# PathologyFoundation/plip

Hardware: NVIDIA H100
Metric: image-text pairs/sec (224x224, 77-tok) (higher is better)
Workload: dtype bf16

## Files before the change

include/plip_b200.h:

```cpp
#ifndef PLIP_B200_H_
#define PLIP_B200_H_

#include <stdint.h>

#ifdef __cplusplus
extern "C" {
#endif

#define PLIP_API __attribute__((visibility("default")))

#define PLIP_B200_ABI_VERSION 5

#define PLIP_IMAGE_SIZE 224
#define PLIP_EMBED_DIM 512
#define PLIP_TEXT_SEQ 77
#define PLIP_VOCAB 49408

typedef struct plip_engine plip_engine_t;

enum plip_pixel_format {
  PLIP_PIX_F32_NCHW = 0,
  PLIP_PIX_BF16_NCHW = 1,
  PLIP_PIX_U8_NHWC = 2
};
// ... 130 lines not shown

typedef struct plip_densenet plip_densenet_t;
PLIP_API int plip_densenet_num_tensors(void);
PLIP_API int plip_densenet_tensor_info(int index, plip_tensor_info_t* info);
PLIP_API uint64_t plip_densenet_blob_bytes(void);
PLIP_API uint64_t plip_densenet_workspace_bytes(int max_micro_batch);
PLIP_API int plip_densenet_create(const void* host_blob, uint64_t blob_bytes, int device, int max_micro_batch,
                                  plip_densenet_t** out);
PLIP_API int plip_densenet_destroy(plip_densenet_t* e);
PLIP_API int plip_densenet_max_micro_batch(const plip_densenet_t* e);
PLIP_API int plip_densenet_encode(plip_densenet_t* e, const void* tiles_dev, int64_t n, float* out_dev, void* stream);

PLIP_API int plip_encode_images_host(plip_engine_t* e, const void* pixels_host, int pixel_format, int64_t n,
                                     float* out_host, int normalize);
PLIP_API int plip_encode_text_host(plip_engine_t* e, const void* ids_host, int ids_dtype,
                                   const void* attention_mask_host, int64_t n, int seq_len,
                                   float* out_host, int normalize);

typedef struct plip_kernel_time {
  char name[48];
  int32_t launches;
  float total_ms;
  double flops;
  double bytes;
} plip_kernel_time_t;
PLIP_API int plip_profile_enable(plip_engine_t* e, int on);
PLIP_API int plip_profile_read(plip_engine_t* e, plip_kernel_time_t* out, int cap, int* count);

PLIP_API int plip_dbg_set_operand_format(int operand_format);
PLIP_API int plip_dbg_gemm(const void* A_bf16, int lda, const void* W_bf16, int ldw, int M, int N, int K,
                           const float* bias, void* out, int ldo, const float* pos, int epilogue, int cluster_size,
                           int block_n, const float* colsum, const float* stats_in, int n_partials, void* xb_out,
                           float* stats_out, void* stream);
PLIP_API int plip_dbg_resize_filter(int in_size, int out_size, int xx, int32_t* k_host, int k_cap, int* xmin,
                                    int* count);
PLIP_API int plip_dbg_resize_filter_bilinear(int in_size, int out_size, int xx, int32_t* k_host, int k_cap, int* xmin,
                                             int* count);
PLIP_API int plip_dbg_text_bucket_plan(const int32_t* lens_host, int64_t n, int seq_len, int32_t* perm_host,
                                       int32_t* bucket_start_host, int32_t* bucket_prefix_host, int cap);
PLIP_API int plip_dbg_rowstats_cast(const float* x, int64_t rows, int dim, void* xb_bf16, float* stats, void* stream);
PLIP_API int plip_dbg_layernorm(const float* x, int64_t rows, int dim, int64_t in_row_stride,
                                const float* gamma, const float* beta, float* out_f32, void* out_bf16,
                                void* stream);
PLIP_API int plip_dbg_attention(const void* qkv_bf16, int64_t n_seq, int seq_len, int heads, int causal,
                                const int32_t* key_mask, void* out_bf16, void* stream);
PLIP_API int plip_dbg_attention_probs(const void* qkv_bf16, int64_t n_seq, int seq_len, int heads, int causal,
                                      const int32_t* key_mask, float* probs_dev, void* stream);
PLIP_API int plip_dbg_densenet_op(int op, const void* in_dev, int lda, int64_t n, int side, int c_in, const void* w_dev,
                                  const float* a_scale, const float* a_shift, const float* e_scale,
                                  const float* e_shift, void* out_dev, int ldo, void* stream);
PLIP_API int plip_dbg_im2col(const void* pixels, int pixel_format, int64_t n, void* out_bf16, void* stream);
PLIP_API int plip_dbg_pos_interp(const float* pos_dev, int grid_h, int grid_w, float* out_dev, void* stream);
PLIP_API int plip_dbg_hidden_states_hw(plip_engine_t* e, const void* pixels_dev, int pixel_format, int64_t n,
                                       int height, int width, int num_layers, float* hidden_dev, void* stream);
PLIP_API int plip_dbg_hidden_states(plip_engine_t* e, int tower, const void* input_dev, int input_format,
                                    const void* attention_mask_dev, int64_t n, int num_layers,
                                    float* hidden_dev, void* stream);

#ifdef __cplusplus
}
#endif
#endif
```

plip_b200/_lib.py:

```python
from __future__ import annotations

import ctypes as C
from pathlib import Path

_PKG = Path(__file__).resolve().parent
LIB_PATH = _PKG / "libplip_b200.so"

_vp = C.c_void_p
_i = C.c_int
_i64 = C.c_int64
_u64 = C.c_uint64
_f = C.c_float
_fp = C.c_void_p


class TensorInfo(C.Structure):

    _fields_ = [
        ("name", C.c_char * 96),
        ("offset", C.c_uint64),
        ("numel", C.c_uint64),
        ("dtype", C.c_int32),
        ("rows", C.c_int32),
        ("cols", C.c_int32),
# ... 62 lines not shown
    "plip_window_background_counts": (_i, [_vp, _i, _i, _i64, _vp, _i64, _i, _vp, _vp]),
    "plip_encode_text": (_i, [_vp, _vp, _i, _vp, _i64, _i, _fp, _i, _vp]),
    "plip_encode_text_prefix": (_i, [_vp, _vp, _i, _vp, _i64, _i, _i, _fp, _i, _vp]),
    "plip_vision_outputs": (_i, [_vp, _vp, _i, _i64, _i, _i, C.POINTER(TowerOutputs), _vp]),
    "plip_text_outputs": (_i, [_vp, _vp, _i, _vp, _i64, _i, C.POINTER(TowerOutputs), _vp]),
    "plip_similarity": (_i, [_fp, _i64, _fp, _i64, _f, _i, _i, _fp, _i64, _vp]),
    "plip_similarity_topk": (_i, [_fp, _i64, _fp, _i64, _f, _i, _i, _i, _vp, _fp, _vp]),
    "plip_l2_normalize": (_i, [_fp, _i64, _i, _vp]),
    "plip_window_mask_counts": (_i, [_vp, _i, _i, _i, _i64, _vp, _i64, _i, _vp, _vp]),
    "plip_resize_crop_u8": (_i, [_vp, _u64, _vp, _i64, _vp, _vp]),
    "plip_resize_crop_bilinear_u8": (_i, [_vp, _u64, _vp, _i64, _vp, _vp]),
    "plip_warp_tiles_u8": (_i, [_vp, _vp, _vp, _i64, _vp]),
    "plip_resize_region_workspace": (_i, [_i, _i, _i, _i, _i, _i, C.POINTER(_u64)]),
    "plip_resize_region_u8": (_i, [_vp, _i64, _i, _i, _i, _i, _vp, _i64, _i, _i, _i, _i, _vp, _u64, _vp]),
    "plip_resize_filter_bounds": (_i, [_i, _i, _vp]),
    "plip_sgd_shuffle_permutation": (_i, [_i64, C.c_uint32, _vp]),
    "plip_sgd_workspace_bytes": (_i, [_i64, _i, _i, C.POINTER(_u64)]),
    "plip_sgd_fit": (_i, [_fp, _i64, _i, _vp, _i, _vp, _i, _vp, _i, _i, C.c_double, _i, _fp, _vp, _vp, _vp, _vp, _u64,
                          _vp]),
    "plip_linear_decision": (_i, [_fp, _i64, _i, _fp, _vp, _i, _fp, _vp, _vp]),
    "plip_densenet_num_tensors": (_i, []),
    "plip_densenet_tensor_info": (_i, [_i, C.POINTER(TensorInfo)]),
    "plip_densenet_blob_bytes": (_u64, []),
    "plip_densenet_workspace_bytes": (_u64, [_i]),
    "plip_densenet_create": (_i, [_vp, _u64, _i, _i, C.POINTER(_vp)]),
    "plip_densenet_destroy": (_i, [_vp]),
    "plip_densenet_max_micro_batch": (_i, [_vp]),
    "plip_densenet_encode": (_i, [_vp, _vp, _i64, _fp, _vp]),
    "plip_encode_images_host": (_i, [_vp, _vp, _i, _i64, _fp, _i]),
    "plip_encode_text_host": (_i, [_vp, _vp, _i, _vp, _i64, _i, _fp, _i]),
    "plip_profile_enable": (_i, [_vp, _i]),
    "plip_profile_read": (_i, [_vp, C.POINTER(KernelTime), _i, C.POINTER(_i)]),
    "plip_dbg_gemm": (_i, [_vp, _i, _vp, _i, _i, _i, _i, _fp, _vp, _i, _fp, _i, _i, _i, _fp, _fp, _i, _vp, _fp, _vp]),
    "plip_dbg_resize_filter": (_i, [_i, _i, _i, _vp, _i, C.POINTER(_i), C.POINTER(_i)]),
    "plip_dbg_resize_filter_bilinear": (_i, [_i, _i, _i, _vp, _i, C.POINTER(_i), C.POINTER(_i)]),
    "plip_dbg_text_bucket_plan": (_i, [_vp, _i64, _i, _vp, _vp, _vp, _i]),
    "plip_dbg_rowstats_cast": (_i, [_fp, _i64, _i, _vp, _fp, _vp]),
    "plip_dbg_layernorm": (_i, [_fp, _i64, _i, _i64, _fp, _fp, _fp, _vp, _vp]),
    "plip_dbg_attention": (_i, [_vp, _i64, _i, _i, _i, _vp, _vp, _vp]),
    "plip_dbg_attention_probs": (_i, [_vp, _i64, _i, _i, _i, _vp, _fp, _vp]),
    "plip_dbg_densenet_op": (_i, [_i, _vp, _i, _i64, _i, _i, _vp, _fp, _fp, _fp, _fp, _vp, _i, _vp]),
    "plip_dbg_im2col": (_i, [_vp, _i, _i64, _vp, _vp]),
    "plip_dbg_hidden_states": (_i, [_vp, _i, _vp, _i, _vp, _i64, _i, _fp, _vp]),
    "plip_dbg_pos_interp": (_i, [_fp, _i, _i, _fp, _vp]),
    "plip_dbg_hidden_states_hw": (_i, [_vp, _vp, _i, _i64, _i, _i, _i, _fp, _vp]),
}

_LIB = None


def lib(strict: bool = True) -> C.CDLL:
    global _LIB
    if _LIB is not None:
        return _LIB
    if not LIB_PATH.exists():
        raise RuntimeError(
            f"{LIB_PATH} is missing: build it with `python -m plip_b200.build` "
            "(plip_b200 has no CPU fallback; the sm_90a CUDA library is the product)."
        )
    dll = C.CDLL(str(LIB_PATH))
    missing = []
    for name, (res, args) in SIGNATURES.items():
        try:
            fn = getattr(dll, name)
        except AttributeError:
            missing.append(name)
# ... 18 lines not shown
```

plip_b200/csrc/engine.cu:

```cuda
#include "kernels.cuh"

#include <stdlib.h>
#include <string.h>

#include <array>
#include <map>
#include <string>
#include <tuple>
#include <vector>

namespace plip {
const char* get_last_error();

namespace {

struct Spec {
  std::string name;
  int dtype;
  int rows, cols, fused;
  uint64_t offset, numel;
};

void add(std::vector<Spec>& v, const std::string& name, int dtype, int rows, int cols, int fused = 0) {
  Spec s;
// ... 1216 lines not shown
  }
  for (int k = 0; k < nb; ++k) {
    const int64_t r0 = start[k], cnt = start[k + 1] - start[k];
    if (cnt <= 0) continue;
    if (int rc = plip_encode_text_prefix(e, d_ids + (size_t)r0 * row_bytes, ids_dtype,
                                         d_mask ? d_mask + (size_t)r0 * row_bytes : nullptr, cnt, seq_len, prefix[k],
                                         e->d_out + r0 * kProj, normalize, e->s_compute)) return rc;
  }
  std::vector<float> tmp((size_t)n * kProj);
  PLIP_CUDA_CHECK(cudaMemcpyAsync(tmp.data(), e->d_out, (size_t)n * kProj * 4, cudaMemcpyDeviceToHost, e->s_compute));
  PLIP_CUDA_CHECK(cudaStreamSynchronize(e->s_compute));
  for (int64_t i = 0; i < n; ++i)
    memcpy(out_host + (size_t)perm[(size_t)i] * kProj, tmp.data() + (size_t)i * kProj, (size_t)kProj * 4);
  return 0;
}

PLIP_API int plip_dbg_text_bucket_plan(const int32_t* lens_host, int64_t n, int seq_len, int32_t* perm_host,
                                       int32_t* bucket_start_host, int32_t* bucket_prefix_host, int cap) {
  if (!lens_host || !bucket_start_host || !bucket_prefix_host || n <= 0 || seq_len < 1 || seq_len > kTxtSeq || cap < 1) {
    set_last_error("plip_dbg_text_bucket_plan: bad argument");
    return -2;
  }
  return plan_text_buckets(lens_host, n, seq_len, perm_host, bucket_start_host, bucket_prefix_host, cap);
}

static int g_dbg_f16 = 0;
PLIP_API int plip_dbg_set_operand_format(int operand_format) {
  PLIP_REQUIRE(operand_format == PLIP_OPERAND_BF16 || operand_format == PLIP_OPERAND_FP16,
               "plip_dbg_set_operand_format: unknown operand format %d", operand_format);
  g_dbg_f16 = operand_format == PLIP_OPERAND_FP16 ? 1 : 0;
  return 0;
}

PLIP_API int plip_dbg_gemm(const void* A_bf16, int lda, const void* W_bf16, int ldw, int M, int N, int K,
                           const float* bias, void* out, int ldo, const float* pos, int epilogue, int cluster_size,
                           int block_n, const float* colsum, const float* stats_in, int n_partials, void* xb_out,
                           float* stats_out, void* stream) {
  GemmArgs g;
  g.A = static_cast<const __nv_bfloat16*>(A_bf16); g.lda = lda;
  g.W = static_cast<const __nv_bfloat16*>(W_bf16); g.ldw = ldw;
  g.M = M; g.N = N; g.K = K;
  g.bias = bias; g.out = out; g.ldo = ldo; g.pos = pos; g.epi = epilogue;
  g.colsum = colsum; g.stats_in = reinterpret_cast<const float2*>(stats_in); g.n_partials = n_partials;
  g.xb_out = static_cast<__nv_bfloat16*>(xb_out); g.stats_out = reinterpret_cast<float2*>(stats_out);
  g.force_cg = cluster_size; g.force_bn = block_n;
  g.f16 = g_dbg_f16;
  return launch_gemm(g, static_cast<cudaStream_t>(stream));
}

PLIP_API int plip_dbg_rowstats_cast(const float* x, int64_t rows, int dim, void* xb_bf16, float* stats, void* stream) {
  return launch_rowstats_cast(x, rows, dim, static_cast<__nv_bfloat16*>(xb_bf16), reinterpret_cast<float2*>(stats),
                              g_dbg_f16, static_cast<cudaStream_t>(stream));
}

PLIP_API int plip_dbg_layernorm(const float* x, int64_t rows, int dim, int64_t in_row_stride, const float* gamma,
                                const float* beta, float* out_f32, void* out_bf16, void* stream) {
  return launch_layernorm(x, nullptr, in_row_stride, rows, dim, gamma, beta, out_f32,
                          static_cast<__nv_bfloat16*>(out_bf16), g_dbg_f16, static_cast<cudaStream_t>(stream));
}

PLIP_API int plip_dbg_attention(const void* qkv_bf16, int64_t n_seq, int seq_len, int heads, int causal,
                                const int32_t* key_mask, void* out_bf16, void* stream) {
  return launch_attention(static_cast<const __nv_bfloat16*>(qkv_bf16), n_seq, seq_len, heads, causal != 0, key_mask,
                          static_cast<__nv_bfloat16*>(out_bf16), g_dbg_f16, static_cast<cudaStream_t>(stream));
}

PLIP_API int plip_dbg_attention_probs(const void* qkv_bf16, int64_t n_seq, int seq_len, int heads, int causal,
                                      const int32_t* key_mask, float* probs_dev, void* stream) {
  return launch_attention_probs(static_cast<const __nv_bfloat16*>(qkv_bf16), n_seq, seq_len, heads, causal != 0,
                                key_mask, probs_dev, g_dbg_f16, static_cast<cudaStream_t>(stream));
}

PLIP_API int plip_dbg_im2col(const void* pixels, int pixel_format, int64_t n, void* out_bf16, void* stream) {
  return launch_im2col(pixels, pixel_format, n, kImage, kImage, static_cast<__nv_bfloat16*>(out_bf16), g_dbg_f16,
                       static_cast<cudaStream_t>(stream));
}

PLIP_API int plip_dbg_pos_interp(const float* pos_dev, int grid_h, int grid_w, float* out_dev, void* stream) {
  return launch_pos_interp(pos_dev, grid_h, grid_w, out_dev, static_cast<cudaStream_t>(stream));
}
// ... 16 lines not shown
```

plip_b200/csrc/gemm.cuh:

```cuda
#pragma once
#include "common.cuh"

namespace plip {

enum GemmEpilogue : int {
  EPI_BIAS_BF16 = 0,
  EPI_BIAS_GELU_BF16 = 1,
  EPI_BIAS_RESID_F32 = 2,
  EPI_PATCH_F32 = 3,
  EPI_F32 = 4,
  EPI_LN_BIAS_BF16 = 5,
  EPI_LN_BIAS_GELU_BF16 = 6,
  EPI_NULL = 7,
  EPI_SIM_F32 = 8,
  EPI_COUNT = 9
};

constexpr int kStatSlots = 8;

struct GemmArgs {
  const __nv_bfloat16* A = nullptr;
  int lda = 0;
  const __nv_bfloat16* W = nullptr;
  int ldw = 0;
  int M = 0, N = 0, K = 0;
  const float* bias = nullptr;
  const float* rowscale = nullptr;
  void* out = nullptr;
  int ldo = 0;
  const float* pos = nullptr;
  int patches = kPatches;
  int seq = kVisSeq;
  const float* colsum = nullptr;
  const float2* stats_in = nullptr;
  int n_partials = 0;
  __nv_bfloat16* xb_out = nullptr;
  float2* stats_out = nullptr;
  int* n_tiles_used = nullptr;
  int epi = EPI_F32;
  int f16 = 0;
  int force_cg = 0;
  int force_bn = 0;
};

int launch_gemm(const GemmArgs& g, cudaStream_t stream);

}
```

plip_b200/csrc/gemm_wgmma.cu:

```cuda
#include "gemm.cuh"
#include "wgmma.cuh"

#include <stdio.h>
#include <stdlib.h>

namespace plip {

namespace {

constexpr int BM = 64;
constexpr int BK = 64;
constexpr int kThreads = 288;
constexpr int kConsumerWarps = 8;
constexpr uint32_t A_STAGE = BM * BK * 2;
constexpr uint32_t kStoreStageBytes = 16 * 128;

constexpr int x_boxes(int BN, int EPI) {
  return EPI != EPI_BIAS_RESID_F32 ? 2 : BN == 192 ? 3 : 2;
}

template <int BN, int EPI>
struct Cfg {
  static constexpr uint32_t B_STAGE = BN * BK * 2;
  static constexpr uint32_t STAGE = A_STAGE + B_STAGE;
  static constexpr int XBOXES = x_boxes(BN, EPI);
  static constexpr uint32_t EPI_BYTES = kConsumerWarps * XBOXES * kStoreStageBytes;
  static constexpr uint32_t BAR_BYTES = EPI == EPI_BIAS_RESID_F32 ? 512 : 256;
  static constexpr uint32_t ALIGN_SLACK = 1024;
  static constexpr int kMaxStages = (227 * 1024 - BAR_BYTES - EPI_BYTES - ALIGN_SLACK) / STAGE;
  static constexpr int STAGES = kMaxStages > 8 ? 8 : kMaxStages;
  static constexpr uint32_t SMEM_BYTES = STAGES * STAGE + EPI_BYTES + BAR_BYTES + ALIGN_SLACK;
};

struct GemmDev {
  int M, N, K;
  const float* bias;
  const float* rowscale;
  void* out;
  int ldo;
  const float* pos;
  int patches, seq;
  const float* colsum;
  const float2* stats_in;
  int n_partials;
  __nv_bfloat16* xb_out;
  float2* stats_out;
};

template <bool F16, int BN>
__device__ __forceinline__ void wgmma_ss(float (&d)[BN / 2], uint64_t adesc, uint64_t bdesc, uint32_t scale_d) {
  if constexpr (BN == 128) wgmma_ss_n128<F16>(d, adesc, bdesc, scale_d);
  else if constexpr (BN == 192) wgmma_ss_n192<F16>(d, adesc, bdesc, scale_d);
  else wgmma_ss_n256<F16>(d, adesc, bdesc, scale_d);
}

__device__ __forceinline__ float2 ln_row_terms(const GemmDev& p, int grow) {
  float s1 = 0.f, s2 = 0.f;
#pragma unroll
  for (int j = 0; j < kStatSlots; ++j) {
    const float2 t = (grow < p.M && j < p.n_partials) ? __ldg(p.stats_in + static_cast<size_t>(grow) * kStatSlots + j)
                                                      : make_float2(0.f, 0.f);
    s1 += t.x;
    s2 += t.y;
  }
  const float inv_k = 1.0f / static_cast<float>(p.K);
  const float mean = s1 * inv_k;
  const float rstd = rsqrtf(fmaxf(s2 * inv_k - mean * mean, 0.f) + kLnEps);
  return make_float2(-rstd * mean, rstd);
}

template <int BN, int EPI, bool F16>
__device__ __forceinline__ void epilogue_warp(const GemmDev& p, const CUtensorMap* tmC, float (&d)[BN / 2], uint32_t stage_smem,
                                              uint32_t& stage_sel, uint32_t xbar, int row_base, int col_base, int n_blk, int lane,
                                              float2 ln0, float2 ln1) {
  constexpr bool LN_FOLD = (EPI == EPI_LN_BIAS_BF16 || EPI == EPI_LN_BIAS_GELU_BF16);
  constexpr bool GELU = (EPI == EPI_BIAS_GELU_BF16 || EPI == EPI_LN_BIAS_GELU_BF16);
  constexpr bool HAS_BIAS = (EPI == EPI_BIAS_BF16 || EPI == EPI_BIAS_GELU_BF16 || EPI == EPI_BIAS_RESID_F32 || LN_FOLD);
  constexpr bool OUT_BF16 = (EPI == EPI_BIAS_BF16 || EPI == EPI_BIAS_GELU_BF16 || LN_FOLD);
  const int q = lane & 3, rr = lane >> 2;
  const int row0 = row_base + rr, row1 = row0 + 8;

  if constexpr (EPI == EPI_NULL) {
    float acc = 0.f;
#pragma unroll
    for (int i = 0; i < BN / 2; ++i) acc += d[i];
    if (acc == 1.2345e30f && p.M < 0) reinterpret_cast<float*>(p.out)[0] = acc;
  } else if constexpr (OUT_BF16) {
#pragma unroll
    for (int blk = 0; blk < BN / 64; ++blk) {
      const uint32_t buf = stage_smem + (stage_sel & 1u) * kStoreStageBytes;
      ++stage_sel;
      if (lane == 0) tma_store_wait_read_but_one();
      __syncwarp();
#pragma unroll
      for (int jj = 0; jj < 8; ++jj) {
        const int j = blk * 8 + jj;
        const int col = col_base + 8 * j + 2 * q;
        const float2 b = __ldg(reinterpret_cast<const float2*>(p.bias + col));
        float v00 = d[4 * j + 0], v01 = d[4 * j + 1], v10 = d[4 * j + 2], v11 = d[4 * j + 3];
        if constexpr (LN_FOLD) {
          const float2 cs = __ldg(reinterpret_cast<const float2*>(p.colsum + col));
          v00 = fmaf(ln0.y, v00, fmaf(ln0.x, cs.x, b.x));
          v01 = fmaf(ln0.y, v01, fmaf(ln0.x, cs.y, b.y));
          v10 = fmaf(ln1.y, v10, fmaf(ln1.x, cs.x, b.x));
          v11 = fmaf(ln1.y, v11, fmaf(ln1.x, cs.y, b.y));
        } else {
          v00 += b.x; v01 += b.y; v10 += b.x; v11 += b.y;
        }
        if constexpr (GELU) {
          v00 = quick_gelu(v00); v01 = quick_gelu(v01); v10 = quick_gelu(v10); v11 = quick_gelu(v11);
        }
        st_shared_b32(buf + rr * 128 + ((jj ^ rr) << 4) + q * 4, pack_op2<F16>(v00, v01));
        st_shared_b32(buf + (rr + 8) * 128 + ((jj ^ rr) << 4) + q * 4, pack_op2<F16>(v10, v11));
      }
      fence_proxy_async_smem();
      __syncwarp();
      if (lane == 0) {
        tma_store_2d(tmC, buf, col_base + blk * 64, row_base);
        tma_store_commit();
      }
    }
  } else if constexpr (EPI == EPI_BIAS_RESID_F32) {
    constexpr int kChunkCols = 32;
    constexpr int kChunks = BN / kChunkCols;
    constexpr int NB = x_boxes(BN, EPI);
    static_assert(kChunks % NB == 0, "every tile must start at staging block 0");
    constexpr int kUses = kChunks / NB;
    const bool ok0 = row0 < p.M, ok1 = row1 < p.M;
    const bool emit = p.xb_out != nullptr;
    const size_t o0 = static_cast<size_t>(ok0 ? row0 : 0) * p.ldo + col_base + 2 * q;
    const size_t o1 = o0 + 8 * static_cast<size_t>(p.ldo);
    uint32_t ph0 = 0;
    if constexpr (kUses % 2 != 0) ph0 = stage_sel++ & 1u;
    auto fetch = [&](int c) {
// ... 85 lines not shown
      o1 = static_cast<size_t>(b1 * p.seq + 1 + (r1 - b1 * p.patches)) * p.ldo;
      q0 = static_cast<size_t>(1 + (r0 - b0 * p.patches)) * p.N;
      q1 = static_cast<size_t>(1 + (r1 - b1 * p.patches)) * p.N;
    }
#pragma unroll
    for (int j = 0; j < BN / 8; ++j) {
      const int col = col_base + 8 * j + 2 * q;
      float2 v0 = make_float2(d[4 * j + 0], d[4 * j + 1]), v1 = make_float2(d[4 * j + 2], d[4 * j + 3]);
      if constexpr (HAS_BIAS) {
        const float2 b = __ldg(reinterpret_cast<const float2*>(p.bias + col));
        v0.x += b.x; v0.y += b.y; v1.x += b.x; v1.y += b.y;
      }
      if constexpr (EPI == EPI_SIM_F32) {
        const float2 cs = __ldg(reinterpret_cast<const float2*>(p.bias + col));
        if (ok0) *reinterpret_cast<float2*>(out + o0 + col) = make_float2(v0.x * rs0 * cs.x, v0.y * rs0 * cs.y);
        if (ok1) *reinterpret_cast<float2*>(out + o1 + col) = make_float2(v1.x * rs1 * cs.x, v1.y * rs1 * cs.y);
      } else if constexpr (EPI == EPI_PATCH_F32) {
        if (ok0) {
          const float2 e = __ldg(reinterpret_cast<const float2*>(p.pos + q0 + col));
          *reinterpret_cast<float2*>(out + o0 + col) = make_float2(v0.x + e.x, v0.y + e.y);
        }
        if (ok1) {
          const float2 e = __ldg(reinterpret_cast<const float2*>(p.pos + q1 + col));
          *reinterpret_cast<float2*>(out + o1 + col) = make_float2(v1.x + e.x, v1.y + e.y);
        }
      } else {
        if (ok0) *reinterpret_cast<float2*>(out + o0 + col) = v0;
        if (ok1) *reinterpret_cast<float2*>(out + o1 + col) = v1;
      }
    }
  }
}

template <int CG, int BN, int EPI, bool F16>
__global__ void __launch_bounds__(kThreads, 1)
gemm_kernel(const __grid_constant__ CUtensorMap tmA, const __grid_constant__ CUtensorMap tmB,
            const __grid_constant__ CUtensorMap tmC, const GemmDev p) {
  using C = Cfg<BN, EPI>;
  constexpr int STAGES = C::STAGES;
  extern __shared__ uint8_t smem_raw[];
  const uint32_t smem_base = (smem_u32(smem_raw) + 1023u) & ~1023u;
  const uint32_t epi_base = smem_base + STAGES * C::STAGE;
  const uint32_t bar_base = epi_base + C::EPI_BYTES;
  auto full_bar = [&](int s) { return bar_base + 8u * s; };
  auto empty_bar = [&](int s) { return bar_base + 8u * (STAGES + s); };
  const uint32_t resid_bar = bar_base + 8u * (2 * STAGES);
  static_assert(8 * (2 * STAGES + (EPI == EPI_BIAS_RESID_F32 ? C::XBOXES * kConsumerWarps : 0)) <= C::BAR_BYTES,
                "barrier area too small");

  const int warp = threadIdx.x >> 5;
  const int lane = threadIdx.x & 31;
  const int wg = warp >> 2;
  const uint32_t cta_rank = (CG > 1) ? cluster_ctarank() : 0u;

  if (threadIdx.x == 0) {
    tma_prefetch_desc(&tmA);
    tma_prefetch_desc(&tmB);
    for (int s = 0; s < STAGES; ++s) {
      mbar_init(full_bar(s), 1);
      mbar_init(empty_bar(s), CG);
    }
    if constexpr (EPI == EPI_BIAS_RESID_F32) {
      tma_prefetch_desc(&tmC);
      for (int i = 0; i < C::XBOXES * kConsumerWarps; ++i) mbar_init(resid_bar + 8u * i, 1);
    }
    fence_mbar_init();
  }
  if constexpr (CG > 1) cluster_sync_all(); else __syncthreads();

  const int num_n_blk = p.N / BN;
  const int num_m_blk = (p.M + BM * CG - 1) / (BM * CG);
  const int num_tiles = num_m_blk * num_n_blk;
  const int num_kb = p.K / BK;
  const int tile0 = blockIdx.x / CG;
  const int tile_step = gridDim.x / CG;
  const int my_tiles = (num_tiles - tile0 + tile_step - 1) / tile_step;

  if (wg == 2) {
    if (lane == 0) {
      int s = 0;
      uint32_t ph = 0;
      for (int t = tile0; t < num_tiles; t += tile_step) {
        const int m0 = ((t / num_n_blk) * CG + cta_rank) * BM;
        const int n0 = (t % num_n_blk) * BN;
        for (int kb = 0; kb < num_kb; ++kb) {
          mbar_wait(empty_bar(s), ph ^ 1u);
          const uint32_t sa = smem_base + s * C::STAGE;
          const uint32_t sb = sa + A_STAGE;
          mbar_arrive_expect_tx(full_bar(s), C::STAGE);
          tma_load_2d(sa, &tmA, full_bar(s), kb * BK, m0);
          if constexpr (CG == 1) {
            tma_load_2d(sb, &tmB, full_bar(s), kb * BK, n0);
          } else {
            tma_load_2d_mc(sb + cta_rank * (C::B_STAGE / 2), &tmB, full_bar(s), kb * BK, n0 + cta_rank * (BN / 2), 0x3);
          }
          if (++s == STAGES) { s = 0; ph ^= 1u; }
        }
      }
    }
    __syncwarp();
  } else {
    const int wtid = threadIdx.x & 127;
    auto release = [&](int s) {
      if (wtid == 0) mbar_arrive(empty_bar(s));
      if constexpr (CG > 1) {
        if (wtid == 32) mbar_arrive_cluster(mapa_shared(empty_bar(s), cta_rank ^ 1u));
      }
    };
    float d[BN / 2];
    int s = 0;
    uint32_t ph = 0;
    auto skip_tile = [&]() {
      s += num_kb;
      ph ^= static_cast<uint32_t>(s / STAGES) & 1u;
      s %= STAGES;
    };
    uint32_t stage_sel = 0;
    const uint32_t my_turn = 1u + wg, other_turn = 2u - wg;
    const int rounds = (my_tiles + 1) / 2;
    if (wg == 1) skip_tile();
    for (int r = 0; r < rounds; ++r) {
      const int i = 2 * r + wg;
      const int t = tile0 + i * tile_step;
      const int n_blk = t % num_n_blk;
      const int m0 = ((t / num_n_blk) * CG + cta_rank) * BM;
      const int wrow = m0 + (warp & 3) * 16;
      float2 ln0 = make_float2(0.f, 1.f), ln1 = make_float2(0.f, 1.f);
      if constexpr (EPI == EPI_LN_BIAS_BF16 || EPI == EPI_LN_BIAS_GELU_BF16) {
        if (i < my_tiles) {
          ln0 = ln_row_terms(p, wrow + (lane >> 2));
          ln1 = ln_row_terms(p, wrow + (lane >> 2) + 8);
        }
      }
      if (wg == 1 || r > 0) named_barrier_sync<256>(my_turn);
      if (i >= my_tiles) break;
      int prev = -1;
      for (int kb = 0; kb < num_kb; ++kb) {
        mbar_wait(full_bar(s), ph);
        const uint32_t sa = smem_base + s * C::STAGE;
        const uint64_t adesc = make_smem_desc_sw128(sa, 1024, 16);
        const uint64_t bdesc = make_smem_desc_sw128(sa + A_STAGE, 1024, 16);
        wgmma_pin(d);
        wgmma_fence();
#pragma unroll
        for (int k = 0; k < BK / 16; ++k) wgmma_ss<F16, BN>(d, adesc + 2 * k, bdesc + 2 * k, (kb | k) != 0 ? 1u : 0u);
        wgmma_commit();
        wgmma_wait<1>();
        if (prev >= 0) release(prev);
        prev = s;
        if (++s == STAGES) { s = 0; ph ^= 1u; }
      }
      if (wg == 0 || r + 1 < rounds) named_barrier_arrive<256>(other_turn);
      wgmma_wait<0>();
      wgmma_pin(d);
      release(prev);
      skip_tile();
      epilogue_warp<BN, EPI, F16>(p, &tmC, d, epi_base + warp * C::XBOXES * kStoreStageBytes, stage_sel,
                                  resid_bar + 8u * C::XBOXES * warp, wrow,
                                  n_blk * BN, n_blk, lane, ln0, ln1);
    }
    if (lane == 0) tma_store_wait_all();
    __syncwarp();
  }
  if constexpr (CG > 1) cluster_sync_all();
}

int env_int(const char* name, int dflt) {
  const char* v = getenv(name);
  return v ? atoi(v) : dflt;
}

template <int CG, int BN, int EPI, bool F16>
int launch_inst(const GemmArgs& g, cudaStream_t stream) {
  using C = Cfg<BN, EPI>;
  auto kern = gemm_kernel<CG, BN, EPI, F16>;
  static unsigned long long configured = 0;
  static int max_groups = 0;
  if (first_use_on_device(configured)) {
    PLIP_CUDA_CHECK(cudaFuncSetAttribute(kern, cudaFuncAttributeMaxDynamicSharedMemorySize, (int)C::SMEM_BYTES));
    int dev = 0, sms = 0;
    PLIP_CUDA_CHECK(cudaGetDevice(&dev));
    PLIP_CUDA_CHECK(cudaDeviceGetAttribute(&sms, cudaDevAttrMultiProcessorCount, dev));
    max_groups = sms / CG;
    if (CG >= 2) {
      cudaLaunchConfig_t q = {};
      q.gridDim = dim3(sms / CG * CG);
      q.blockDim = dim3(kThreads);
      q.dynamicSmemBytes = C::SMEM_BYTES;
      cudaLaunchAttribute qa[1];
      qa[0].id = cudaLaunchAttributeClusterDimension;
      qa[0].val.clusterDim.x = CG; qa[0].val.clusterDim.y = 1; qa[0].val.clusterDim.z = 1;
      q.attrs = qa; q.numAttrs = 1;
      int n_clusters = 0;
      PLIP_CUDA_CHECK(cudaOccupancyMaxActiveClusters(&n_clusters, kern, &q));
      if (n_clusters > 0 && n_clusters < max_groups) max_groups = n_clusters;
    }
    PLIP_REQUIRE(max_groups > 0, "launch_gemm: no resident CTA fits (cg=%d bn=%d)", CG, BN);
  }
  CUtensorMap tmA, tmB;
  if (int rc = make_tmap_bf16_2d(&tmA, g.A, g.M, g.K, (uint64_t)g.lda * 2, BM, BK)) return rc;
  if (int rc = make_tmap_bf16_2d(&tmB, g.W, g.N, g.K, (uint64_t)g.ldw * 2, BN / CG, BK)) return rc;
  constexpr bool kOutBf16 = (EPI == EPI_BIAS_BF16 || EPI == EPI_BIAS_GELU_BF16 || EPI == EPI_LN_BIAS_BF16 ||
                             EPI == EPI_LN_BIAS_GELU_BF16);
  CUtensorMap tmC = tmA;
  if (kOutBf16)
    if (int rc = make_tmap_bf16_2d(&tmC, g.out, g.M, g.N, (uint64_t)g.ldo * 2, 16, 64)) return rc;
  if (EPI == EPI_BIAS_RESID_F32)
    if (int rc = make_tmap_bf16_2d(&tmC, g.out, g.M, 2 * (uint64_t)g.N, (uint64_t)g.ldo * 4, 16, 64)) return rc;

  GemmDev p;
  p.M = g.M; p.N = g.N; p.K = g.K;
  p.bias = g.bias; p.rowscale = g.rowscale; p.out = g.out; p.ldo = g.ldo; p.pos = g.pos;
  p.patches = g.patches; p.seq = g.seq;
  p.colsum = g.colsum; p.stats_in = g.stats_in; p.n_partials = g.n_partials;
  p.xb_out = g.xb_out; p.stats_out = g.stats_out;
  if (g.n_tiles_used) *g.n_tiles_used = 2 * (g.N / BN);

  const int num_tiles = ((g.M + BM * CG - 1) / (BM * CG)) * (g.N / BN);
  const int groups = max_groups < num_tiles ? max_groups : num_tiles;
  PLIP_CUDA_CHECK(launch_kernel(kern, dim3(groups * CG), dim3(kThreads), C::SMEM_BYTES, stream, CG, tmA, tmB, tmC, p));
  return 0;
}

template <int CG, int BN, bool F16>
int launch_epi_fmt(const GemmArgs& g, cudaStream_t stream) {
  switch (g.epi) {
    case EPI_BIAS_BF16: return launch_inst<CG, BN, EPI_BIAS_BF16, F16>(g, stream);
    case EPI_BIAS_GELU_BF16: return launch_inst<CG, BN, EPI_BIAS_GELU_BF16, F16>(g, stream);
    case EPI_BIAS_RESID_F32: return launch_inst<CG, BN, EPI_BIAS_RESID_F32, F16>(g, stream);
    case EPI_PATCH_F32: return launch_inst<CG, BN, EPI_PATCH_F32, F16>(g, stream);
    case EPI_F32: return launch_inst<CG, BN, EPI_F32, F16>(g, stream);
    case EPI_LN_BIAS_BF16: return launch_inst<CG, BN, EPI_LN_BIAS_BF16, F16>(g, stream);
    case EPI_LN_BIAS_GELU_BF16: return launch_inst<CG, BN, EPI_LN_BIAS_GELU_BF16, F16>(g, stream);
    case EPI_NULL: return launch_inst<CG, BN, EPI_NULL, F16>(g, stream);
    case EPI_SIM_F32: return launch_inst<CG, BN, EPI_SIM_F32, F16>(g, stream);
    default: set_last_error("launch_gemm: bad epilogue %d", g.epi); return -2;
  }
}
template <int CG, int BN>
int launch_epi(const GemmArgs& g, cudaStream_t stream) {
  return g.f16 ? launch_epi_fmt<CG, BN, true>(g, stream) : launch_epi_fmt<CG, BN, false>(g, stream);
}

}

int launch_gemm(const GemmArgs& g, cudaStream_t stream) {
  PLIP_REQUIRE(g.M > 0 && g.N > 0 && g.K > 0, "launch_gemm: empty problem M=%d N=%d K=%d", g.M, g.N, g.K);
  PLIP_REQUIRE(g.K % BK == 0, "launch_gemm: K=%d must be a multiple of %d", g.K, BK);
  PLIP_REQUIRE(g.N % 128 == 0 || g.N % 192 == 0, "launch_gemm: N=%d must be a multiple of 128 or 192", g.N);
  PLIP_REQUIRE((g.lda % 8) == 0 && (g.ldw % 8) == 0 && (g.ldo % 8) == 0,
               "launch_gemm: leading dimensions must be multiples of 8 elements");
  PLIP_REQUIRE((reinterpret_cast<uintptr_t>(g.A) & 15) == 0 && (reinterpret_cast<uintptr_t>(g.W) & 15) == 0 &&
               (reinterpret_cast<uintptr_t>(g.out) & 15) == 0,
               "launch_gemm: operands must be 16-byte aligned");
  if (g.epi == EPI_LN_BIAS_BF16 || g.epi == EPI_LN_BIAS_GELU_BF16)
    PLIP_REQUIRE(g.colsum && g.stats_in && g.bias && g.n_partials >= 1 && g.n_partials <= kStatSlots,
                 "launch_gemm: LayerNorm-folded epilogue needs colsum, stats and 1..%d partials", kStatSlots);
  if (g.epi == EPI_SIM_F32)
    PLIP_REQUIRE(g.bias && g.rowscale, "launch_gemm: the similarity epilogue needs row and column scales");
  if (g.epi == EPI_PATCH_F32)
    PLIP_REQUIRE(g.patches >= 1 && g.seq == g.patches + 1, "launch_gemm: patch epilogue with %d patches, %d rows",
                 g.patches, g.seq);
  if (g.xb_out || g.stats_out)
    PLIP_REQUIRE(g.epi == EPI_BIAS_RESID_F32 && g.xb_out && g.stats_out,
                 "launch_gemm: xb/stats outputs belong to the residual epilogue");
  static const int env_cg = env_int("PLIP_GEMM_CG", 0);
  static const int env_bn = env_int("PLIP_GEMM_BN", 0);
  int cg = g.force_cg ? g.force_cg : (env_cg ? env_cg : 2);
  int bn = g.force_bn ? g.force_bn : (env_bn ? env_bn : 256);
  if (g.N % bn != 0) bn = 128;
  if (!g.force_bn && g.stats_out && 2 * (g.N / bn) > kStatSlots && g.N % 256 == 0) bn = 256;
  PLIP_REQUIRE((cg == 1 || cg == 2) && (bn == 128 || bn == 256 || (bn == 192 && cg == 2)),
               "launch_gemm: bad config cg=%d bn=%d", cg, bn);
  PLIP_REQUIRE(!g.stats_out || 2 * (g.N / bn) <= kStatSlots, "launch_gemm: N=%d / BN=%d exceeds %d statistics slots",
               g.N, bn, kStatSlots);
  if (cg == 1) return bn == 256 ? launch_epi<1, 256>(g, stream) : launch_epi<1, 128>(g, stream);
  if (bn == 192) return launch_epi<2, 192>(g, stream);
  return bn == 256 ? launch_epi<2, 256>(g, stream) : launch_epi<2, 128>(g, stream);
}

}
```

Baseline: 26740.

## Add cooperative 128-row GEMM schedule for LayerNorm-folded epilogues with smem-staged vectors

Adds a cooperative schedule in which both consumer warpgroups work on one 128-row tile, sharing each B stage, instead of ping-ponging separate 64-row tiles. For LayerNorm-folded epilogues, bias, colsum and per-row statistics are bulk-copied into shared memory by the producer rather than read per thread from global memory. An auto heuristic picks this path for BN=256 LN epilogues when there are enough tiles. The cost is losing the overlap of one warpgroup's epilogue with the other's MMA, plus fewer pipeline stages because of the larger A stage.

```diff
diff --git a/include/plip_b200.h b/include/plip_b200.h
--- a/include/plip_b200.h
+++ b/include/plip_b200.h
@@ -186,6 +186,10 @@
                            const float* bias, void* out, int ldo, const float* pos, int epilogue, int cluster_size,
                            int block_n, const float* colsum, const float* stats_in, int n_partials, void* xb_out,
                            float* stats_out, void* stream);
+PLIP_API int plip_dbg_gemm_sched(const void* A_bf16, int lda, const void* W_bf16, int ldw, int M, int N, int K,
+                                 const float* bias, void* out, int ldo, const float* pos, int epilogue,
+                                 int cluster_size, int block_n, const float* colsum, const float* stats_in,
+                                 int n_partials, void* xb_out, float* stats_out, int schedule, void* stream);
 PLIP_API int plip_dbg_resize_filter(int in_size, int out_size, int xx, int32_t* k_host, int k_cap, int* xmin,
                                     int* count);
 PLIP_API int plip_dbg_resize_filter_bilinear(int in_size, int out_size, int xx, int32_t* k_host, int k_cap, int* xmin,
diff --git a/plip_b200/_lib.py b/plip_b200/_lib.py
--- a/plip_b200/_lib.py
+++ b/plip_b200/_lib.py
@@ -118,6 +118,8 @@
     "plip_profile_enable": (_i, [_vp, _i]),
     "plip_profile_read": (_i, [_vp, C.POINTER(KernelTime), _i, C.POINTER(_i)]),
     "plip_dbg_gemm": (_i, [_vp, _i, _vp, _i, _i, _i, _i, _fp, _vp, _i, _fp, _i, _i, _i, _fp, _fp, _i, _vp, _fp, _vp]),
+    "plip_dbg_gemm_sched": (_i, [_vp, _i, _vp, _i, _i, _i, _i, _fp, _vp, _i, _fp, _i, _i, _i, _fp, _fp, _i, _vp, _fp,
+                                 _i, _vp]),
     "plip_dbg_resize_filter": (_i, [_i, _i, _i, _vp, _i, C.POINTER(_i), C.POINTER(_i)]),
     "plip_dbg_resize_filter_bilinear": (_i, [_i, _i, _i, _vp, _i, C.POINTER(_i), C.POINTER(_i)]),
     "plip_dbg_text_bucket_plan": (_i, [_vp, _i64, _i, _vp, _vp, _vp, _i]),
diff --git a/plip_b200/csrc/engine.cu b/plip_b200/csrc/engine.cu
--- a/plip_b200/csrc/engine.cu
+++ b/plip_b200/csrc/engine.cu
@@ -1272,10 +1272,10 @@
   return 0;
 }
 
-PLIP_API int plip_dbg_gemm(const void* A_bf16, int lda, const void* W_bf16, int ldw, int M, int N, int K,
-                           const float* bias, void* out, int ldo, const float* pos, int epilogue, int cluster_size,
-                           int block_n, const float* colsum, const float* stats_in, int n_partials, void* xb_out,
-                           float* stats_out, void* stream) {
+PLIP_API int plip_dbg_gemm_sched(const void* A_bf16, int lda, const void* W_bf16, int ldw, int M, int N, int K,
+                                 const float* bias, void* out, int ldo, const float* pos, int epilogue,
+                                 int cluster_size, int block_n, const float* colsum, const float* stats_in,
+                                 int n_partials, void* xb_out, float* stats_out, int schedule, void* stream) {
   GemmArgs g;
   g.A = static_cast<const __nv_bfloat16*>(A_bf16); g.lda = lda;
   g.W = static_cast<const __nv_bfloat16*>(W_bf16); g.ldw = ldw;
@@ -1283,9 +1283,17 @@
   g.bias = bias; g.out = out; g.ldo = ldo; g.pos = pos; g.epi = epilogue;
   g.colsum = colsum; g.stats_in = reinterpret_cast<const float2*>(stats_in); g.n_partials = n_partials;
   g.xb_out = static_cast<__nv_bfloat16*>(xb_out); g.stats_out = reinterpret_cast<float2*>(stats_out);
-  g.force_cg = cluster_size; g.force_bn = block_n;
+  g.force_cg = cluster_size; g.force_bn = block_n; g.force_sched = schedule;
   g.f16 = g_dbg_f16;
   return launch_gemm(g, static_cast<cudaStream_t>(stream));
+}
+
+PLIP_API int plip_dbg_gemm(const void* A_bf16, int lda, const void* W_bf16, int ldw, int M, int N, int K,
+                           const float* bias, void* out, int ldo, const float* pos, int epilogue, int cluster_size,
+                           int block_n, const float* colsum, const float* stats_in, int n_partials, void* xb_out,
+                           float* stats_out, void* stream) {
+  return plip_dbg_gemm_sched(A_bf16, lda, W_bf16, ldw, M, N, K, bias, out, ldo, pos, epilogue, cluster_size, block_n,
+                             colsum, stats_in, n_partials, xb_out, stats_out, 0, stream);
 }
 
 PLIP_API int plip_dbg_rowstats_cast(const float* x, int64_t rows, int dim, void* xb_bf16, float* stats, void* stream) {
diff --git a/plip_b200/csrc/gemm.cuh b/plip_b200/csrc/gemm.cuh
--- a/plip_b200/csrc/gemm.cuh
+++ b/plip_b200/csrc/gemm.cuh
@@ -41,6 +41,7 @@
   int f16 = 0;
   int force_cg = 0;
   int force_bn = 0;
+  int force_sched = 0;
 };
 
 int launch_gemm(const GemmArgs& g, cudaStream_t stream);
diff --git a/plip_b200/csrc/gemm_wgmma.cu b/plip_b200/csrc/gemm_wgmma.cu
--- a/plip_b200/csrc/gemm_wgmma.cu
+++ b/plip_b200/csrc/gemm_wgmma.cu
@@ -8,28 +8,37 @@
 
 namespace {
 
-constexpr int BM = 64;
+enum Sched : int { PINGPONG = 0, COOP = 1 };
+
 constexpr int BK = 64;
 constexpr int kThreads = 288;
 constexpr int kConsumerWarps = 8;
-constexpr uint32_t A_STAGE = BM * BK * 2;
 constexpr uint32_t kStoreStageBytes = 16 * 128;
+constexpr uint32_t kWgRows = 64;
 
 constexpr int x_boxes(int BN, int EPI) {
   return EPI != EPI_BIAS_RESID_F32 ? 2 : BN == 192 ? 3 : 2;
 }
 
-template <int BN, int EPI>
+constexpr int kCoopBoxes = 4;
+
+template <int BN, int EPI, int SCHED = PINGPONG>
 struct Cfg {
+  static constexpr int BM = SCHED == COOP ? 2 * kWgRows : kWgRows;
+  static constexpr bool SMEM_VEC = SCHED == COOP && (EPI == EPI_LN_BIAS_BF16 || EPI == EPI_LN_BIAS_GELU_BF16);
+  static constexpr uint32_t VEC_TILE = SMEM_VEC ? 2 * BN * 4 : 0;
+  static constexpr uint32_t STATS_BYTES = SMEM_VEC ? BM * kStatSlots * 8 : 0;
+  static constexpr uint32_t VEC_BYTES = 2 * VEC_TILE + STATS_BYTES;
+  static constexpr uint32_t A_STAGE = BM * BK * 2;
   static constexpr uint32_t B_STAGE = BN * BK * 2;
   static constexpr uint32_t STAGE = A_STAGE + B_STAGE;
-  static constexpr int XBOXES = x_boxes(BN, EPI);
+  static constexpr int XBOXES = SCHED == COOP ? kCoopBoxes : x_boxes(BN, EPI);
   static constexpr uint32_t EPI_BYTES = kConsumerWarps * XBOXES * kStoreStageBytes;
   static constexpr uint32_t BAR_BYTES = EPI == EPI_BIAS_RESID_F32 ? 512 : 256;
   static constexpr uint32_t ALIGN_SLACK = 1024;
-  static constexpr int kMaxStages = (227 * 1024 - BAR_BYTES - EPI_BYTES - ALIGN_SLACK) / STAGE;
+  static constexpr int kMaxStages = (227 * 1024 - BAR_BYTES - EPI_BYTES - VEC_BYTES - ALIGN_SLACK) / STAGE;
   static constexpr int STAGES = kMaxStages > 8 ? 8 : kMaxStages;
-  static constexpr uint32_t SMEM_BYTES = STAGES * STAGE + EPI_BYTES + BAR_BYTES + ALIGN_SLACK;
+  static constexpr uint32_t SMEM_BYTES = STAGES * STAGE + EPI_BYTES + VEC_BYTES + BAR_BYTES + ALIGN_SLACK;
 };
 
 struct GemmDev {
@@ -47,6 +56,11 @@
   float2* stats_out;
 };
 
+__device__ __forceinline__ void bulk_load_1d(uint32_t smem_dst, const void* src, uint32_t bytes, uint32_t bar) {
+  asm volatile("cp.async.bulk.shared::cluster.global.mbarrier::complete_tx::bytes [%0], [%1], %2, [%3];"
+               ::"r"(smem_dst), "l"(reinterpret_cast<uint64_t>(src)), "r"(bytes), "r"(bar) : "memory");
+}
+
 template <bool F16, int BN>
 __device__ __forceinline__ void wgmma_ss(float (&d)[BN / 2], uint64_t adesc, uint64_t bdesc, uint32_t scale_d) {
   if constexpr (BN == 128) wgmma_ss_n128<F16>(d, adesc, bdesc, scale_d);
@@ -54,12 +68,15 @@
   else wgmma_ss_n256<F16>(d, adesc, bdesc, scale_d);
 }
 
-__device__ __forceinline__ float2 ln_row_terms(const GemmDev& p, int grow) {
+template <bool SMEM = false>
+__device__ __forceinline__ float2 ln_row_terms(const GemmDev& p, int grow, uint32_t srow = 0) {
   float s1 = 0.f, s2 = 0.f;
 #pragma unroll
   for (int j = 0; j < kStatSlots; ++j) {
-    const float2 t = (grow < p.M && j < p.n_partials) ? __ldg(p.stats_in + static_cast<size_t>(grow) * kStatSlots + j)
-                                                      : make_float2(0.f, 0.f);
+    const float2 t = (grow < p.M && j < p.n_partials)
+                         ? (SMEM ? ld_shared_f32x2(srow + 8 * j)
+                                 : __ldg(p.stats_in + static_cast<size_t>(grow) * kStatSlots + j))
+                         : make_float2(0.f, 0.f);
     s1 += t.x;
     s2 += t.y;
   }
@@ -69,10 +86,10 @@
   return make_float2(-rstd * mean, rstd);
 }
 
-template <int BN, int EPI, bool F16>
+template <int BN, int EPI, bool F16, int NBUF, bool SMEM_VEC>
 __device__ __forceinline__ void epilogue_warp(const GemmDev& p, const CUtensorMap* tmC, float (&d)[BN / 2], uint32_t stage_smem,
                                               uint32_t& stage_sel, uint32_t xbar, int row_base, int col_base, int n_blk, int lane,
-                                              float2 ln0, float2 ln1) {
+                                              float2 ln0, float2 ln1, uint32_t vec_smem) {
   constexpr bool LN_FOLD = (EPI == EPI_LN_BIAS_BF16 || EPI == EPI_LN_BIAS_GELU_BF16);
   constexpr bool GELU = (EPI == EPI_BIAS_GELU_BF16 || EPI == EPI_LN_BIAS_GELU_BF16);
   constexpr bool HAS_BIAS = (EPI == EPI_BIAS_BF16 || EPI == EPI_BIAS_GELU_BF16 || EPI == EPI_BIAS_RESID_F32 || LN_FOLD);
@@ -86,20 +103,28 @@
     for (int i = 0; i < BN / 2; ++i) acc += d[i];
     if (acc == 1.2345e30f && p.M < 0) reinterpret_cast<float*>(p.out)[0] = acc;
   } else if constexpr (OUT_BF16) {
+    static_assert(NBUF == 2 || NBUF == BN / 64, "staging blocks: two alternating, or one per 64 columns");
 #pragma unroll
     for (int blk = 0; blk < BN / 64; ++blk) {
-      const uint32_t buf = stage_smem + (stage_sel & 1u) * kStoreStageBytes;
+      const uint32_t buf = stage_smem + (stage_sel % NBUF) * kStoreStageBytes;
       ++stage_sel;
-      if (lane == 0) tma_store_wait_read_but_one();
-      __syncwarp();
+      if constexpr (NBUF == 2) {
+        if (lane == 0) tma_store_wait_read_but_one();
+        __syncwarp();
+      } else if (blk == 0) {
+        if (lane == 0) tma_store_wait_read();
+        __syncwarp();
+      }
 #pragma unroll
       for (int jj = 0; jj < 8; ++jj) {
         const int j = blk * 8 + jj;
         const int col = col_base + 8 * j + 2 * q;
-        const float2 b = __ldg(reinterpret_cast<const float2*>(p.bias + col));
+        const float2 b = SMEM_VEC ? ld_shared_f32x2(vec_smem + (8 * j + 2 * q) * 4)
+                                  : __ldg(reinterpret_cast<const float2*>(p.bias + col));
         float v00 = d[4 * j + 0], v01 = d[4 * j + 1], v10 = d[4 * j + 2], v11 = d[4 * j + 3];
         if constexpr (LN_FOLD) {
-          const float2 cs = __ldg(reinterpret_cast<const float2*>(p.colsum + col));
+          const float2 cs = SMEM_VEC ? ld_shared_f32x2(vec_smem + (BN + 8 * j + 2 * q) * 4)
+                                     : __ldg(reinterpret_cast<const float2*>(p.colsum + col));
           v00 = fmaf(ln0.y, v00, fmaf(ln0.x, cs.x, b.x));
           v01 = fmaf(ln0.y, v01, fmaf(ln0.x, cs.y, b.y));
           v10 = fmaf(ln1.y, v10, fmaf(ln1.x, cs.x, b.x));
@@ -251,16 +276,20 @@
   }
 }
 
-template <int CG, int BN, int EPI, bool F16>
+template <int CG, int BN, int EPI, bool F16, int SCHED>
 __global__ void __launch_bounds__(kThreads, 1)
 gemm_kernel(const __grid_constant__ CUtensorMap tmA, const __grid_constant__ CUtensorMap tmB,
             const __grid_constant__ CUtensorMap tmC, const GemmDev p) {
-  using C = Cfg<BN, EPI>;
+  using C = Cfg<BN, EPI, SCHED>;
   constexpr int STAGES = C::STAGES;
+  constexpr int BM = C::BM;
+  static_assert(SCHED == PINGPONG || (BN == 256 && EPI != EPI_BIAS_RESID_F32), "cooperative schedule: BN 256, 16-bit stores");
   extern __shared__ uint8_t smem_raw[];
   const uint32_t smem_base = (smem_u32(smem_raw) + 1023u) & ~1023u;
   const uint32_t epi_base = smem_base + STAGES * C::STAGE;
-  const uint32_t bar_base = epi_base + C::EPI_BYTES;
+  const uint32_t vec_base = epi_base + C::EPI_BYTES;
+  const uint32_t stats_base = vec_base + 2 * C::VEC_TILE;
+  const uint32_t bar_base = vec_base + C::VEC_BYTES;
   auto full_bar = [&](int s) { return bar_base + 8u * s; };
   auto empty_bar = [&](int s) { return bar_base + 8u * (STAGES + s); };
   const uint32_t resid_bar = bar_base + 8u * (2 * STAGES);
@@ -277,7 +306,7 @@
     tma_prefetch_desc(&tmB);
     for (int s = 0; s < STAGES; ++s) {
       mbar_init(full_bar(s), 1);
-      mbar_init(empty_bar(s), CG);
+      mbar_init(empty_bar(s), (SCHED == COOP ? 2 : 1) * CG);
     }
     if constexpr (EPI == EPI_BIAS_RESID_F32) {
       tma_prefetch_desc(&tmC);
@@ -299,14 +328,25 @@
     if (lane == 0) {
       int s = 0;
       uint32_t ph = 0;
-      for (int t = tile0; t < num_tiles; t += tile_step) {
+      for (int t = tile0, i = 0; t < num_tiles; t += tile_step, ++i) {
         const int m0 = ((t / num_n_blk) * CG + cta_rank) * BM;
         const int n0 = (t % num_n_blk) * BN;
         for (int kb = 0; kb < num_kb; ++kb) {
           mbar_wait(empty_bar(s), ph ^ 1u);
           const uint32_t sa = smem_base + s * C::STAGE;
-          const uint32_t sb = sa + A_STAGE;
-          mbar_arrive_expect_tx(full_bar(s), C::STAGE);
+          const uint32_t sb = sa + C::A_STAGE;
+          const int stat_rows = C::SMEM_VEC && kb == 0 ? max(0, min(BM, p.M - m0)) : 0;
+          mbar_arrive_expect_tx(full_bar(s), C::STAGE + (kb == 0 ? C::VEC_TILE : 0u) + stat_rows * kStatSlots * 8);
+          if constexpr (C::SMEM_VEC) {
+            if (kb == 0) {
+              const uint32_t vb = vec_base + (i & 1) * C::VEC_TILE;
+              bulk_load_1d(vb, p.bias + n0, BN * 4, full_bar(s));
+              bulk_load_1d(vb + BN * 4, p.colsum + n0, BN * 4, full_bar(s));
+              if (stat_rows > 0)
+                bulk_load_1d(stats_base, p.stats_in + static_cast<size_t>(m0) * kStatSlots, stat_rows * kStatSlots * 8,
+                             full_bar(s));
+            }
+          }
           tma_load_2d(sa, &tmA, full_bar(s), kb * BK, m0);
           if constexpr (CG == 1) {
             tma_load_2d(sb, &tmB, full_bar(s), kb * BK, n0);
@@ -329,36 +369,13 @@
     float d[BN / 2];
     int s = 0;
     uint32_t ph = 0;
-    auto skip_tile = [&]() {
-      s += num_kb;
-      ph ^= static_cast<uint32_t>(s / STAGES) & 1u;
-      s %= STAGES;
-    };
-    uint32_t stage_sel = 0;
-    const uint32_t my_turn = 1u + wg, other_turn = 2u - wg;
-    const int rounds = (my_tiles + 1) / 2;
-    if (wg == 1) skip_tile();
-    for (int r = 0; r < rounds; ++r) {
-      const int i = 2 * r + wg;
-      const int t = tile0 + i * tile_step;
-      const int n_blk = t % num_n_blk;
-      const int m0 = ((t / num_n_blk) * CG + cta_rank) * BM;
-      const int wrow = m0 + (warp & 3) * 16;
-      float2 ln0 = make_float2(0.f, 1.f), ln1 = make_float2(0.f, 1.f);
-      if constexpr (EPI == EPI_LN_BIAS_BF16 || EPI == EPI_LN_BIAS_GELU_BF16) {
-        if (i < my_tiles) {
-          ln0 = ln_row_terms(p, wrow + (lane >> 2));
-          ln1 = ln_row_terms(p, wrow + (lane >> 2) + 8);
-        }
-      }
-      if (wg == 1 || r > 0) named_barrier_sync<256>(my_turn);
-      if (i >= my_tiles) break;
+    auto issue_tile = [&](uint32_t a_off) {
       int prev = -1;
       for (int kb = 0; kb < num_kb; ++kb) {
         mbar_wait(full_bar(s), ph);
         const uint32_t sa = smem_base + s * C::STAGE;
-        const uint64_t adesc = make_smem_desc_sw128(sa, 1024, 16);
-        const uint64_t bdesc = make_smem_desc_sw128(sa + A_STAGE, 1024, 16);
+        const uint64_t adesc = make_smem_desc_sw128(sa + a_off, 1024, 16);
+        const uint64_t bdesc = make_smem_desc_sw128(sa + C::A_STAGE, 1024, 16);
         wgmma_pin(d);
         wgmma_fence();
 #pragma unroll
@@ -369,14 +386,66 @@
         prev = s;
         if (++s == STAGES) { s = 0; ph ^= 1u; }
       }
-      if (wg == 0 || r + 1 < rounds) named_barrier_arrive<256>(other_turn);
-      wgmma_wait<0>();
-      wgmma_pin(d);
-      release(prev);
-      skip_tile();
-      epilogue_warp<BN, EPI, F16>(p, &tmC, d, epi_base + warp * C::XBOXES * kStoreStageBytes, stage_sel,
-                                  resid_bar + 8u * C::XBOXES * warp, wrow,
-                                  n_blk * BN, n_blk, lane, ln0, ln1);
+      return prev;
+    };
+    auto ln_terms = [&](int wrow, float2& ln0, float2& ln1) {
+      if constexpr (EPI == EPI_LN_BIAS_BF16 || EPI == EPI_LN_BIAS_GELU_BF16) {
+        ln0 = ln_row_terms(p, wrow + (lane >> 2));
+        ln1 = ln_row_terms(p, wrow + (lane >> 2) + 8);
+      }
+    };
+    uint32_t stage_sel = 0;
+    if constexpr (SCHED == COOP) {
+      for (int t = tile0, i = 0; t < num_tiles; t += tile_step, ++i) {
+        const int n_blk = t % num_n_blk;
+        const int m0 = ((t / num_n_blk) * CG + cta_rank) * BM;
+        const int wrow = m0 + wg * kWgRows + (warp & 3) * 16;
+        float2 ln0 = make_float2(0.f, 1.f), ln1 = make_float2(0.f, 1.f);
+        if constexpr (C::SMEM_VEC) {
+          mbar_wait(full_bar(s), ph);
+          const int r0 = wrow - m0 + (lane >> 2);
+          ln0 = ln_row_terms<true>(p, wrow + (lane >> 2), stats_base + r0 * kStatSlots * 8);
+          ln1 = ln_row_terms<true>(p, wrow + (lane >> 2) + 8, stats_base + (r0 + 8) * kStatSlots * 8);
+        } else {
+          ln_terms(wrow, ln0, ln1);
+        }
+        const int last = issue_tile(wg * kWgRows * BK * 2);
+        wgmma_wait<0>();
+        wgmma_pin(d);
+        release(last);
+        epilogue_warp<BN, EPI, F16, C::XBOXES, C::SMEM_VEC>(p, &tmC, d, epi_base + warp * C::XBOXES * kStoreStageBytes,
+                                                            stage_sel, 0u, wrow, n_blk * BN, n_blk, lane, ln0, ln1,
+                                                            vec_base + (i & 1) * C::VEC_TILE);
+      }
+    } else {
+      auto skip_tile = [&]() {
+        s += num_kb;
+        ph ^= static_cast<uint32_t>(s / STAGES) & 1u;
+        s %= STAGES;
+      };
+      const uint32_t my_turn = 1u + wg, other_turn = 2u - wg;
+      const int rounds = (my_tiles + 1) / 2;
+      if (wg == 1) skip_tile();
+      for (int r = 0; r < rounds; ++r) {
+        const int i = 2 * r + wg;
+        const int t = tile0 + i * tile_step;
+        const int n_blk = t % num_n_blk;
+        const int m0 = ((t / num_n_blk) * CG + cta_rank) * BM;
+        const int wrow = m0 + (warp & 3) * 16;
+        float2 ln0 = make_float2(0.f, 1.f), ln1 = make_float2(0.f, 1.f);
+        if (i < my_tiles) ln_terms(wrow, ln0, ln1);
+        if (wg == 1 || r > 0) named_barrier_sync<256>(my_turn);
+        if (i >= my_tiles) break;
+        const int last = issue_tile(0u);
+        if (wg == 0 || r + 1 < rounds) named_barrier_arrive<256>(other_turn);
+        wgmma_wait<0>();
+        wgmma_pin(d);
+        release(last);
+        skip_tile();
+        epilogue_warp<BN, EPI, F16, C::XBOXES, false>(p, &tmC, d, epi_base + warp * C::XBOXES * kStoreStageBytes,
+                                                      stage_sel, resid_bar + 8u * C::XBOXES * warp, wrow,
+                                                      n_blk * BN, n_blk, lane, ln0, ln1, 0u);
+      }
     }
     if (lane == 0) tma_store_wait_all();
     __syncwarp();
@@ -389,10 +458,11 @@
   return v ? atoi(v) : dflt;
 }
 
-template <int CG, int BN, int EPI, bool F16>
+template <int CG, int BN, int EPI, bool F16, int SCHED>
 int launch_inst(const GemmArgs& g, cudaStream_t stream) {
-  using C = Cfg<BN, EPI>;
-  auto kern = gemm_kernel<CG, BN, EPI, F16>;
+  using C = Cfg<BN, EPI, SCHED>;
+  constexpr int BM = C::BM;
+  auto kern = gemm_kernel<CG, BN, EPI, F16, SCHED>;
   static unsigned long long configured = 0;
   static int max_groups = 0;
   if (first_use_on_device(configured)) {
@@ -414,7 +484,13 @@
       PLIP_CUDA_CHECK(cudaOccupancyMaxActiveClusters(&n_clusters, kern, &q));
       if (n_clusters > 0 && n_clusters < max_groups) max_groups = n_clusters;
     }
-    PLIP_REQUIRE(max_groups > 0, "launch_gemm: no resident CTA fits (cg=%d bn=%d)", CG, BN);
+    PLIP_REQUIRE(max_groups > 0, "launch_gemm: no resident CTA fits (cg=%d bn=%d sched=%d)", CG, BN, SCHED);
+  }
+  if constexpr (C::SMEM_VEC) {
+    PLIP_REQUIRE(g.K / BK >= C::STAGES, "launch_gemm: the cooperative schedule needs K >= %d (K=%d)", C::STAGES * BK, g.K);
+    PLIP_REQUIRE(((reinterpret_cast<uintptr_t>(g.bias) | reinterpret_cast<uintptr_t>(g.colsum) |
+                   reinterpret_cast<uintptr_t>(g.stats_in)) & 15) == 0,
+                 "launch_gemm: the cooperative schedule needs 16-byte aligned bias, colsum and statistics");
   }
   CUtensorMap tmA, tmB;
   if (int rc = make_tmap_bf16_2d(&tmA, g.A, g.M, g.K, (uint64_t)g.lda * 2, BM, BK)) return rc;
@@ -444,21 +520,48 @@
 template <int CG, int BN, bool F16>
 int launch_epi_fmt(const GemmArgs& g, cudaStream_t stream) {
   switch (g.epi) {
-    case EPI_BIAS_BF16: return launch_inst<CG, BN, EPI_BIAS_BF16, F16>(g, stream);
-    case EPI_BIAS_GELU_BF16: return launch_inst<CG, BN, EPI_BIAS_GELU_BF16, F16>(g, stream);
-    case EPI_BIAS_RESID_F32: return launch_inst<CG, BN, EPI_BIAS_RESID_F32, F16>(g, stream);
-    case EPI_PATCH_F32: return launch_inst<CG, BN, EPI_PATCH_F32, F16>(g, stream);
-    case EPI_F32: return launch_inst<CG, BN, EPI_F32, F16>(g, stream);
-    case EPI_LN_BIAS_BF16: return launch_inst<CG, BN, EPI_LN_BIAS_BF16, F16>(g, stream);
-    case EPI_LN_BIAS_GELU_BF16: return launch_inst<CG, BN, EPI_LN_BIAS_GELU_BF16, F16>(g, stream);
-    case EPI_NULL: return launch_inst<CG, BN, EPI_NULL, F16>(g, stream);
-    case EPI_SIM_F32: return launch_inst<CG, BN, EPI_SIM_F32, F16>(g, stream);
+    case EPI_BIAS_BF16: return launch_inst<CG, BN, EPI_BIAS_BF16, F16, PINGPONG>(g, stream);
+    case EPI_BIAS_GELU_BF16: return launch_inst<CG, BN, EPI_BIAS_GELU_BF16, F16, PINGPONG>(g, stream);
+    case EPI_BIAS_RESID_F32: return launch_inst<CG, BN, EPI_BIAS_RESID_F32, F16, PINGPONG>(g, stream);
+    case EPI_PATCH_F32: return launch_inst<CG, BN, EPI_PATCH_F32, F16, PINGPONG>(g, stream);
+    case EPI_F32: return launch_inst<CG, BN, EPI_F32, F16, PINGPONG>(g, stream);
+    case EPI_LN_BIAS_BF16: return launch_inst<CG, BN, EPI_LN_BIAS_BF16, F16, PINGPONG>(g, stream);
+    case EPI_LN_BIAS_GELU_BF16: return launch_inst<CG, BN, EPI_LN_BIAS_GELU_BF16, F16, PINGPONG>(g, stream);
+    case EPI_NULL: return launch_inst<CG, BN, EPI_NULL, F16, PINGPONG>(g, stream);
+    case EPI_SIM_F32: return launch_inst<CG, BN, EPI_SIM_F32, F16, PINGPONG>(g, stream);
     default: set_last_error("launch_gemm: bad epilogue %d", g.epi); return -2;
   }
 }
 template <int CG, int BN>
 int launch_epi(const GemmArgs& g, cudaStream_t stream) {
   return g.f16 ? launch_epi_fmt<CG, BN, true>(g, stream) : launch_epi_fmt<CG, BN, false>(g, stream);
+}
+
+template <int CG, bool F16>
+int launch_coop_fmt(const GemmArgs& g, cudaStream_t stream) {
+  switch (g.epi) {
+    case EPI_LN_BIAS_BF16: return launch_inst<CG, 256, EPI_LN_BIAS_BF16, F16, COOP>(g, stream);
+    case EPI_LN_BIAS_GELU_BF16: return launch_inst<CG, 256, EPI_LN_BIAS_GELU_BF16, F16, COOP>(g, stream);
+    case EPI_NULL: return launch_inst<CG, 256, EPI_NULL, F16, COOP>(g, stream);
+    default: set_last_error("launch_gemm: no cooperative kernel for epilogue %d", g.epi); return -2;
+  }
+}
+template <int CG>
+int launch_coop(const GemmArgs& g, cudaStream_t stream) {
+  return g.f16 ? launch_coop_fmt<CG, true>(g, stream) : launch_coop_fmt<CG, false>(g, stream);
+}
+
+bool auto_coop(const GemmArgs& g, int cg, int bn) {
+  if (bn != 256 || (g.epi != EPI_LN_BIAS_BF16 && g.epi != EPI_LN_BIAS_GELU_BF16)) return false;
+  if (g.K / BK < Cfg<256, EPI_LN_BIAS_BF16, COOP>::STAGES ||
+      ((reinterpret_cast<uintptr_t>(g.bias) | reinterpret_cast<uintptr_t>(g.colsum) |
+        reinterpret_cast<uintptr_t>(g.stats_in)) & 15) != 0)
+    return false;
+  int dev = 0, sms = 0;
+  if (cudaGetDevice(&dev) != cudaSuccess || cudaDeviceGetAttribute(&sms, cudaDevAttrMultiProcessorCount, dev) != cudaSuccess)
+    return false;
+  const long long coop_tiles = static_cast<long long>((g.M + 128 * cg - 1) / (128 * cg)) * (g.N / 256);
+  return coop_tiles >= 2LL * (sms / cg);
 }
 
 }
@@ -493,6 +596,11 @@
                "launch_gemm: bad config cg=%d bn=%d", cg, bn);
   PLIP_REQUIRE(!g.stats_out || 2 * (g.N / bn) <= kStatSlots, "launch_gemm: N=%d / BN=%d exceeds %d statistics slots",
                g.N, bn, kStatSlots);
+  PLIP_REQUIRE(g.force_sched >= 0 && g.force_sched <= 2, "launch_gemm: bad schedule %d", g.force_sched);
+  if (g.force_sched == 2 || (g.force_sched == 0 && auto_coop(g, cg, bn))) {
+    PLIP_REQUIRE(bn == 256, "launch_gemm: the cooperative schedule needs BN 256 (bn=%d)", bn);
+    return cg == 1 ? launch_coop<1>(g, stream) : launch_coop<2>(g, stream);
+  }
   if (cg == 1) return bn == 256 ? launch_epi<1, 256>(g, stream) : launch_epi<1, 128>(g, stream);
   if (bn == 192) return launch_epi<2, 192>(g, stream);
   return bn == 256 ? launch_epi<2, 256>(g, stream) : launch_epi<2, 128>(g, stream);
```

Result: faster. 27170 (median of 6 runs) (+1.6%).
